# GrafikXxxxxxxYyyyyyyyyyy/StableDiffusion

Hardware: AMD Instinct MI355X
Metric: denoise-loop latents/s (512px, 50-step DDIM, batch 4) (higher is better)
Workload: dtype f16; 1 GPU; SD1.5 512x512, 50-step DDIM, batch 4/GPU, CFG on (UNet batch 8), UNet + VAE decode HIP kernels; global_batch=4, parallelism=dp1

## Files before the change

### stablediffusion_amd/build.py

```python
from __future__ import annotations

import os
import subprocess
import sys
from concurrent.futures import ThreadPoolExecutor

HERE = os.path.dirname(os.path.abspath(__file__))
CSRC = os.path.join(HERE, "csrc")
OUT = os.path.join(HERE, "libsd_engine.so")
SOURCES = ["igemm.hip", "igemm2.hip", "igemm3.hip", "wsgemm.hip", "pgemm.hip", "ffn.hip", "edge.hip", "norm.hip", "attention.hip", "ip_attention.hip", "controlnet.hip", "misc.hip", "probe.hip", "runtime.cpp", "unet.cpp", "controlnet.cpp", "vae.cpp", "clip.cpp", "capi.cpp"]
FLAGS = ["-O3", "--offload-arch=gfx950", "-fPIC", "-std=c++17", "-Wall", "-Wno-unused-function",
         "-ffp-contract=fast", "-mllvm", "-amdgpu-mfma-vgpr-form"]


def _stale(target, deps):
    if not os.path.exists(target):
        return True
    t = os.path.getmtime(target)
    return any(os.path.getmtime(d) > t for d in deps)


def build(force: bool = False, verbose: bool = False) -> str:
    hipcc = os.environ.get("HIPCC", "/opt/rocm/bin/hipcc")
    objdir = os.path.join(HERE, "build")
    os.makedirs(objdir, exist_ok=True)
    headers = [os.path.join(CSRC, f) for f in os.listdir(CSRC) if f.endswith((".h", ".inc"))]
    headers.append(os.path.join(os.path.dirname(HERE), "include", "sd_engine.h"))
    jobs = []
    objs = []
    for src in SOURCES:
        s = os.path.join(CSRC, src)
        o = os.path.join(objdir, src + ".o")
        objs.append(o)
        if force or _stale(o, [s] + headers):
            jobs.append([hipcc, *FLAGS, "-x", "hip", "-c", s, "-o", o])

    def run(cmd):
        if verbose:
            print(" ".join(cmd), flush=True)
        r = subprocess.run(cmd, capture_output=True, text=True)
        if r.returncode != 0:
            raise RuntimeError("build failed: %s\n%s\n%s" % (" ".join(cmd), r.stdout, r.stderr))
        if verbose and r.stderr.strip():
            print(r.stderr, file=sys.stderr)

    if jobs:
        with ThreadPoolExecutor(max_workers=min(8, len(jobs))) as ex:
            list(ex.map(run, jobs))
    if jobs or force or _stale(OUT, objs):
        run([hipcc, "--offload-arch=gfx950", "-shared", "-fPIC", "-o", OUT, *objs])
    return OUT


if __name__ == "__main__":
    print(build(force="--force" in sys.argv, verbose=True))
```

### stablediffusion_amd/csrc/attention.hip

```cpp
#include <cstdlib>

#include "kernels.h"

namespace sd {
namespace {

[[maybe_unused]] constexpr float kRescaleThreshold = 8.0f;

constexpr int odd32_bytes(int bytes) { return ((((bytes + 31) / 32) | 1)) * 32; }
constexpr int k_row_halves(int D) { return D == 40 ? 40 : odd32_bytes((D + 31) / 32 * 32 * 2) / 2; }

typedef __fp16 fp16x2 __attribute__((ext_vector_type(2)));

__device__ __forceinline__ unsigned pack_rtz(float a, float b) {
    return __builtin_bit_cast(unsigned, __builtin_amdgcn_cvt_pkrtz(a, b));
}

template <int D, int QT, int KT, bool PRESC, int NWV = 4>
__global__ __launch_bounds__(64 * NWV) void attn_kernel(const half_t* __restrict__ q,
                                                   const half_t* __restrict__ k,
                                                   const half_t* __restrict__ v,
                                                   half_t* __restrict__ out, int Tq, int Tk_all,
                                                   int heads, long ldq, long ldk, long ldv,
                                                   long ldo, float scale_log2e, int causal, int qblocks) {
    static_assert(KT == 64 || KT == 128, "keys per tile");
#if defined(__HIP_DEVICE_COMPILE__)
    constexpr int NSUB = KT / 16;
    constexpr int NKK = KT / 32;
    constexpr int DK = (D + 31) / 32 * 32;
    constexpr int KS = DK / 32;
    constexpr int DT = (D + 15) / 16 + ((D % 16 == 0 && D <= 64) ? 1 : 0);
    constexpr int KSTR = k_row_halves(D);
    constexpr int VSTR = odd32_bytes(DT * 16 * 2) / 2;
    constexpr int CH = D / 8;
    constexpr int NCH = KT * CH;
    constexpr bool ONES = DT * 16 > D;
    constexpr bool PREFETCH = D <= 160;
    constexpr int QB = 16 * QT * NWV;
    constexpr int NTH = 64 * NWV;

    constexpr int TILE_HALVES = KT * (KSTR + VSTR);
    extern __shared__ __attribute__((aligned(16))) char smem[];
    half_t* sK = reinterpret_cast<half_t*>(smem);
    half_t* sV = sK + KT * KSTR;

    const int tid = threadIdx.x, lane = tid & 63, wave = tid >> 6;
    const int fr = lane & 15, fq = lane >> 4;
    const int bid = xcd_remap(blockIdx.x, gridDim.x);
    const int bh = bid / qblocks, qblk = bid - bh * qblocks;
    const int b = bh / heads, h = bh - b * heads;
    const int q0 = qblk * QB + wave * (16 * QT);

    const half_t* qb = q + (long)b * Tq * ldq + h * D;
    int Tk = Tk_all;
    if (causal && qblk * QB + QB < Tk) Tk = qblk * QB + QB;
    const half_t* kb = k + (long)b * Tk_all * ldk + h * D;
    const half_t* vb = v + (long)b * Tk_all * ldv + h * D;

    constexpr int KPAD = KSTR - D, VPAD = VSTR - D;
#pragma unroll
    for (int bufi = 0; bufi < (PREFETCH ? 2 : 1); ++bufi) {
        if constexpr (KPAD > 0) {
            for (int idx = tid; idx < KT * KPAD; idx += NTH) {
                const int r = idx / KPAD, c = D + idx - r * KPAD;
                sK[bufi * TILE_HALVES + r * KSTR + c] = (half_t)0.f;
            }
        }
        if constexpr (VPAD > 0) {
            for (int idx = tid; idx < KT * VPAD; idx += NTH) {
                const int r = idx / VPAD, c = D + idx - r * VPAD;
                sV[bufi * TILE_HALVES + r * VSTR + c] = (ONES && c == D) ? (half_t)1.f : (half_t)0.f;
            }
        }
    }

    h8 qf[QT][KS];
#pragma unroll
    for (int t = 0; t < QT; ++t) {
        const int qi = q0 + t * 16 + fr;
#pragma unroll
        for (int ks = 0; ks < KS; ++ks) {
            const int c = ks * 32 + fq * 8;
            h8 val = {0, 0, 0, 0, 0, 0, 0, 0};
            if (qi < Tq && c < D) val = *reinterpret_cast<const h8*>(qb + (long)qi * ldq + c);
            qf[t][ks] = val;
        }
    }

    f4 o[DT][QT];
#pragma unroll
    for (int i = 0; i < DT; ++i)
#pragma unroll
        for (int t = 0; t < QT; ++t) o[i][t] = f4{0.f, 0.f, 0.f, 0.f};
    float mrun[QT], lrun[QT];
#pragma unroll
    for (int t = 0; t < QT; ++t) { mrun[t] = PRESC ? 0.f : -INFINITY; lrun[t] = 0.f; }
    f4 negm[QT];
#pragma unroll
    for (int t = 0; t < QT; ++t) negm[t] = f4{0.f, 0.f, 0.f, 0.f};

    constexpr unsigned kOOB = 0x80000000u;
    constexpr int SPRK = KSTR / 8, SPRV = VSTR / 8;
    constexpr int NP = SPRK + SPRV, NPW = (NP + NWV - 1) / NWV;
    const int wavu = __builtin_amdgcn_readfirstlane(wave);
    __amdgpu_buffer_rsrc_t rk = __builtin_amdgcn_make_buffer_rsrc(const_cast<half_t*>(kb), 0, 0x7fffffff, 0x00020000);
    __amdgpu_buffer_rsrc_t rv = __builtin_amdgcn_make_buffer_rsrc(const_cast<half_t*>(vb), 0, 0x7fffffff, 0x00020000);
    int p_row[NPW], p_off[NPW];
#pragma unroll
    for (int j = 0; j < NPW; ++j) {
        const int q = wavu + NWV * j;
        const bool isk = q < SPRK;
        const int spr = isk ? SPRK : SPRV;
        const int p = (isk ? q : q - SPRK) * 64 + lane;
        const int r = p / spr, c = p - r * spr;
        p_row[j] = r;
        p_off[j] = c < CH ? (int)((r * (isk ? ldk : ldv) + c * 8) * 2) : -1;
    }
    auto issue_tile = [&](int bufi, int kt0) {
        half_t* dK = sK + bufi * TILE_HALVES;
        half_t* dV = sV + bufi * TILE_HALVES;
        const unsigned kbase = (unsigned)((long)kt0 * ldk * 2), vbase = (unsigned)((long)kt0 * ldv * 2);
        const int lim = Tk - kt0;
#pragma unroll
        for (int j = 0; j < NPW; ++j) {
            const int q = wavu + NWV * j;
            if (q < NP && p_off[j] >= 0) {
                const bool isk = q < SPRK;
                const unsigned voff = p_row[j] < lim ? (isk ? kbase : vbase) + (unsigned)p_off[j] : kOOB;
                half_t* dst = isk ? dK + q * 512 : dV + (q - SPRK) * 512;
                if (isk)
                    __builtin_amdgcn_raw_ptr_buffer_load_lds(rk, (__attribute__((address_space(3))) void*)dst, 16, voff, 0, 0, 0);
                else
                    __builtin_amdgcn_raw_ptr_buffer_load_lds(rv, (__attribute__((address_space(3))) void*)dst, 16, voff, 0, 0, 0);
            }
        }
    };
    if (PREFETCH) {
        __syncthreads();
        issue_tile(0, 0);
        asm volatile("s_waitcnt vmcnt(0)" ::: "memory");
        __syncthreads();
    }

    int cur = 0;
    for (int kt0 = 0; kt0 < Tk; kt0 += KT) {
        if (PREFETCH) {
            if (kt0 + KT < Tk) issue_tile(cur ^ 1, kt0 + KT);
        } else {
            __syncthreads();
            for (int idx = tid; idx < NCH; idx += NTH) {
                const int r = idx / CH, c = (idx - r * CH) * 8;
                h8 kv = {0, 0, 0, 0, 0, 0, 0, 0}, vv = {0, 0, 0, 0, 0, 0, 0, 0};
                if (kt0 + r < Tk) {
                    kv = *reinterpret_cast<const h8*>(kb + (long)(kt0 + r) * ldk + c);
                    vv = *reinterpret_cast<const h8*>(vb + (long)(kt0 + r) * ldv + c);
                }
                *reinterpret_cast<h8*>(sK + r * KSTR + c) = kv;
                *reinterpret_cast<h8*>(sV + r * VSTR + c) = vv;
            }
            __syncthreads();
        }
        const half_t* cK = sK + cur * TILE_HALVES;
        const half_t* cV = sV + cur * TILE_HALVES;

        f4 s[NSUB][QT];
#pragma unroll
        for (int ksub = 0; ksub < NSUB; ++ksub)
#pragma unroll
            for (int t = 0; t < QT; ++t) s[ksub][t] = PRESC ? negm[t] : f4{0.f, 0.f, 0.f, 0.f};
#pragma unroll
        for (int ks = 0; ks < KS; ++ks) {
#pragma unroll
            for (int ksub = 0; ksub < NSUB; ++ksub) {
                const h8 kf = *reinterpret_cast<const h8*>(cK + (ksub * 16 + fr) * KSTR + ks * 32 + fq * 8);
#pragma unroll
                for (int t = 0; t < QT; ++t)
                    s[ksub][t] = __builtin_amdgcn_mfma_f32_16x16x32_f16(kf, qf[t][ks], s[ksub][t], 0, 0, 0);
            }
        }
        if (kt0 + KT > Tk) {
#pragma unroll
            for (int ksub = 0; ksub < NSUB; ++ksub)
#pragma unroll
                for (int j = 0; j < 4; ++j)
                    if (kt0 + ksub * 16 + fq * 4 + j >= Tk) {
#pragma unroll
                        for (int t = 0; t < QT; ++t) s[ksub][t][j] = -INFINITY;
                    }
        }

        if (causal && kt0 + KT - 1 > q0) {
#pragma unroll
            for (int t = 0; t < QT; ++t) {
                const int qi = q0 + t * 16 + fr;
#pragma unroll
                for (int ksub = 0; ksub < NSUB; ++ksub)
#pragma unroll
                    for (int j = 0; j < 4; ++j)
                        if (kt0 + ksub * 16 + fq * 4 + j > qi) s[ksub][t][j] = -INFINITY;
            }
        }

        unsigned pf[QT][NKK][4];
        if constexpr (PRESC) {
            float mx[QT];
            bool grow = kt0 == 0;
#pragma unroll
            for (int t = 0; t < QT; ++t) {
                float m = -INFINITY;
#pragma unroll
                for (int ksub = 0; ksub < NSUB; ++ksub)
#pragma unroll
                    for (int j = 0; j < 4; ++j) m = fmaxf(m, s[ksub][t][j]);
                mx[t] = m;
                grow |= m > kRescaleThreshold;
            }
            if (__any(grow)) {
#pragma unroll
                for (int t = 0; t < QT; ++t) {
                    mx[t] = fmaxf(mx[t], __shfl_xor(mx[t], 16));
                    mx[t] = fmaxf(mx[t], __shfl_xor(mx[t], 32));
                    const float delta = kt0 == 0 ? mx[t] : fmaxf(mx[t], 0.f);
                    const float alpha = kt0 == 0 ? 1.f : __builtin_amdgcn_exp2f(-delta);
                    mrun[t] += delta;
                    negm[t] = f4{-mrun[t], -mrun[t], -mrun[t], -mrun[t]};
#pragma unroll
                    for (int i = 0; i < DT; ++i) o[i][t] *= alpha;
                    lrun[t] *= alpha;
#pragma unroll
                    for (int ksub = 0; ksub < NSUB; ++ksub) s[ksub][t] -= delta;
                }
            }
#pragma unroll
            for (int t = 0; t < QT; ++t) {
                float psum = 0.f;
#pragma unroll
                for (int ksub = 0; ksub < NSUB; ++ksub) {
                    float p[4];
#pragma unroll
                    for (int j = 0; j < 4; ++j) {
                        p[j] = __builtin_amdgcn_exp2f(s[ksub][t][j]);
                        if (!ONES) psum += p[j];
                    }
                    pf[t][ksub >> 1][(ksub & 1) * 2] = pack_rtz(p[0], p[1]);
                    pf[t][ksub >> 1][(ksub & 1) * 2 + 1] = pack_rtz(p[2], p[3]);
                }
                if (!ONES) lrun[t] += psum;
            }
        } else {
            bool grow = false;
            float mx[QT];
    #pragma unroll
            for (int t = 0; t < QT; ++t) {
                float m = -INFINITY;
    #pragma unroll
                for (int ksub = 0; ksub < NSUB; ++ksub)
    #pragma unroll
                    for (int j = 0; j < 4; ++j) m = fmaxf(m, s[ksub][t][j]);
                m = fmaxf(m, __shfl_xor(m, 16));
                m = fmaxf(m, __shfl_xor(m, 32));
                mx[t] = m * scale_log2e;
                grow |= mx[t] > mrun[t] + kRescaleThreshold;
            }
            if (__any(grow)) {
    #pragma unroll
                for (int t = 0; t < QT; ++t) {
                    const float mnew = fmaxf(mrun[t], mx[t]);
                    const float alpha = __builtin_amdgcn_exp2f(mrun[t] - mnew);
                    mrun[t] = mnew;
                    lrun[t] *= alpha;
    #pragma unroll
                    for (int i = 0; i < DT; ++i) o[i][t] *= alpha;
                }
            }
    #pragma unroll
            for (int t = 0; t < QT; ++t) {
                const float nm = -mrun[t];
                float psum = 0.f;
    #pragma unroll
                for (int ksub = 0; ksub < NSUB; ++ksub) {
                    float p[4];
    #pragma unroll
                    for (int j = 0; j < 4; ++j) {
                        p[j] = __builtin_amdgcn_exp2f(__builtin_fmaf(s[ksub][t][j], scale_log2e, nm));
                        if (!ONES) psum += p[j];
                    }
                    pf[t][ksub >> 1][(ksub & 1) * 2] = pack_rtz(p[0], p[1]);
                    pf[t][ksub >> 1][(ksub & 1) * 2 + 1] = pack_rtz(p[2], p[3]);
                }
                if (!ONES) lrun[t] += psum;
            }
        }

#pragma unroll
        for (int i = 0; i < DT; ++i) {
#pragma unroll
            for (int kk = 0; kk < NKK; ++kk) {
                const half_t* a0 = cV + (kk * 32 + fq * 4 + (fr >> 2)) * VSTR + i * 16 + (fr & 3) * 4;
                const s4v lo = __builtin_amdgcn_ds_read_tr16_b64_v4i16(
                    (__attribute__((address_space(3))) s4v*)(a0));
                const s4v hi = __builtin_amdgcn_ds_read_tr16_b64_v4i16(
                    (__attribute__((address_space(3))) s4v*)(a0 + 16 * VSTR));
                union { struct { s4v a, b; } p; h8 v; } u;
                u.p.a = lo; u.p.b = hi;
#pragma unroll
                for (int t = 0; t < QT; ++t) {
                    union { unsigned w[4]; h8 v; } pb;
#pragma unroll
                    for (int e = 0; e < 4; ++e) pb.w[e] = pf[t][kk][e];
                    o[i][t] = __builtin_amdgcn_mfma_f32_16x16x32_f16(u.v, pb.v, o[i][t], 0, 0, 0);
                }
            }
        }
        if (PREFETCH) {
            asm volatile("s_waitcnt vmcnt(0)" ::: "memory");
            __syncthreads();
            cur ^= 1;
        }
    }

    half_t* ob = out + (long)b * Tq * ldo + h * D;
#pragma unroll
    for (int t = 0; t < QT; ++t) {
        float l;
        if (ONES) {
            constexpr int LT = D / 16, LQ = (D % 16) / 4, LJ = D % 4;
            l = __shfl(o[LT][t][LJ], LQ * 16 + fr);
        } else {
            l = lrun[t];
            l += __shfl_xor(l, 16);
            l += __shfl_xor(l, 32);
        }
        const float inv = 1.0f / l;
        const int qi = q0 + t * 16 + fr;
#pragma unroll
        for (int i = 0; i < DT; ++i) {
            const int dd = i * 16 + fq * 4;
            if (qi < Tq && dd < D) {
                const f4 val = o[i][t] * inv;
                h4 w = {(half_t)val[0], (half_t)val[1], (half_t)val[2], (half_t)val[3]};
                *reinterpret_cast<h4*>(ob + (long)qi * ldo + dd) = w;
            }
        }
    }
#endif
}

template <int D, int QT, int KT, bool PRESC, int NWV = 4>
int launch_attn(const half_t* q, const half_t* k, const half_t* v, half_t* out, int B, int Tq, int Tk,
                int heads, long ldq, long ldk, long ldv, long ldo, int causal, bool q_has_scale, hipStream_t s) {
    constexpr int DK = (D + 31) / 32 * 32;
    constexpr int DT = (D + 15) / 16 + ((D % 16 == 0 && D <= 64) ? 1 : 0);
    constexpr size_t lds = (size_t)KT * (k_row_halves(D) * 2 + odd32_bytes(DT * 16 * 2)) * (D <= 160 ? 2 : 1);
    static PerDeviceOnce attr_once;
    if (attr_once.first()) {
        SD_HIP_CHECK(hipFuncSetAttribute(reinterpret_cast<const void*>(&attn_kernel<D, QT, KT, PRESC, NWV>),
                                         hipFuncAttributeMaxDynamicSharedMemorySize, (int)lds));
    }
    const float scale_log2e = q_has_scale ? 1.0f : 1.4426950408889634f / sqrtf((float)D);
    const int qblocks = cdiv(Tq, 16 * QT * NWV);
    hipLaunchKernelGGL((attn_kernel<D, QT, KT, PRESC, NWV>), dim3(qblocks * B * heads), dim3(64 * NWV), lds, s, q, k, v,
                       out, Tq, Tk, heads, ldq, ldk, ldv, ldo, scale_log2e, causal, qblocks);
    SD_HIP_CHECK(hipGetLastError());
    return 0;
}

}

bool attention_supported(int d) {
    return d == 32 || d == 40 || d == 64 || d == 80 || d == 128 || d == 160 || d == 512;
}

int launch_attention(const half_t* q, const half_t* k, const half_t* v, half_t* out, int B, int Tq,
                     int Tk, int heads, int d, long ldq, long ldk, long ldv, long ldo, hipStream_t s, int causal,
                     int prescaled) {
    if ((ldq | ldk | ldv | ldo) % 8 != 0) { set_error("attention: row strides must be multiples of 8"); return 1; }
    if (Tk <= 0 || Tq <= 0) return 0;
#define SD_ATTN_CASE(DD, QQ, KK, FAST) \
    case DD: return (prescaled && FAST) \
        ? launch_attn<DD, QQ, KK, FAST>(q, k, v, out, B, Tq, Tk, heads, ldq, ldk, ldv, ldo, causal, true, s) \
        : launch_attn<DD, QQ, KK, false>(q, k, v, out, B, Tq, Tk, heads, ldq, ldk, ldv, ldo, causal, prescaled != 0, s)
    static const int nwv = getenv("SD_ATTN_NWV") ? atoi(getenv("SD_ATTN_NWV")) : 8;
    if (d == 40 && prescaled && !causal && nwv == 8 && (long)cdiv(Tq, 512) * B * heads >= 512)
        return launch_attn<40, 4, 64, true, 8>(q, k, v, out, B, Tq, Tk, heads, ldq, ldk, ldv, ldo, causal, true, s);
    static const int nwv80 = getenv("SD_ATTN_NWV80") ? atoi(getenv("SD_ATTN_NWV80")) : 8;
    if (nwv80 == 8 && !causal && d == 80 && (long)cdiv(Tq, 256) * B * heads >= 256)
        return launch_attn<80, 2, 64, false, 8>(q, k, v, out, B, Tq, Tk, heads, ldq, ldk, ldv, ldo, causal, prescaled != 0, s);
    if (d == 160 && (long)cdiv(Tq, 128) * B * heads < 256)
        return launch_attn<160, 1, 64, false>(q, k, v, out, B, Tq, Tk, heads, ldq, ldk, ldv, ldo, causal, prescaled != 0, s);
    switch (d) {
        SD_ATTN_CASE(32, 2, 64, true);
        SD_ATTN_CASE(40, 4, 64, true);
        SD_ATTN_CASE(64, 2, 64, false);
        SD_ATTN_CASE(80, 2, 64, false);
        SD_ATTN_CASE(128, 2, 64, false);
        SD_ATTN_CASE(160, 2, 64, false);
        SD_ATTN_CASE(512, 1, 64, false);
        default:
            set_error("attention: unsupported head dim " + std::to_string(d));
            return 4;
    }
#undef SD_ATTN_CASE
}

}
```

### stablediffusion_amd/csrc/kernels.h

```cpp
#pragma once
#include "common.h"

namespace sd {

struct IGemmParams {
    const half_t* x; long ldx;
    const half_t* w;
    const float* bias;
    const float* rowadd; int rowadd_ld;
    const half_t* res; long ldres;
    half_t* y; long ldy;
    int N, H, W, Cin;
    int OH, OW, Cout;
    int KS, stride, pad, up;
    int M, K;
    int geglu;
    int mfast = 0;
    int act = 0;
    float* rowstat_out = nullptr;
    int rowstat_parts = 0;
    const float* ln_stat = nullptr;
    int ln_parts = 0, ln_C = 0, ln_part_w = 0;
    float ln_eps = 0.f;
    const float* ln_wsum = nullptr;
    float* gnstat_out = nullptr;
    int gn_groups = 0;
    const float* gni_part = nullptr;
    int gni_S = 0;
    long gni_rows = 0;
    int gni_groups = 0;
    float gni_eps = 0.f;
    int gni_silu = 0;
    const float* gni_gb = nullptr;
    int dbg_unchecked = 0;
    float acc_scale = 1.f, bias_scale = 1.f;
};
bool igemm2_gn_fusable(const IGemmParams& p, int groups);
bool igemm2_scales_ok(const IGemmParams& p);
bool igemm2_emits_gnstats(const IGemmParams& p, int groups, int* rows);
bool igemm2_emits_rowstats(const IGemmParams& p, int* parts, int* part_w);
int launch_igemm(const IGemmParams& p, hipStream_t s);
const char* igemm_variant(const IGemmParams& p);
bool igemm2_supported(const IGemmParams& p);
void igemm2_pick(const IGemmParams& p, int* variant, int* splits);
const char* igemm2_name(int variant);
long igemm2_partial_floats(const IGemmParams& p);
int launch_igemm2(const IGemmParams& p, float* partial, hipStream_t s);
constexpr int kKindPgemmGeglu = 100;
int igemm2_launch_kind(const IGemmParams& p, bool have_partial);
void igemm2_force(int variant, int splits);
bool igemm3_supported(const IGemmParams& p);
int launch_igemm3(const IGemmParams& p, int mfast, hipStream_t s);
constexpr int kWeightRowPad = 256;
bool wsgemm_supported(const IGemmParams& p);
int wsgemm_rowstat_parts(const IGemmParams& p);
int launch_wsgemm(const IGemmParams& p, hipStream_t s);
bool pgemm_geglu_supported(const IGemmParams& p);
int launch_pgemm_geglu(const IGemmParams& p, hipStream_t s);

struct FfnParams {
    const half_t* x; long ldx;
    half_t* y; long ldy;
    const half_t* w1; const float* b1; const float* wsum1; int w1_rows;
    const half_t* w2; const float* b2; int w2_rows;
    const float* ln_stat; int ln_parts; float ln_eps;
    int M, C, hidden;
    int ln_part_w;
};
bool ffn_fused_supported(const FfnParams& p);
int launch_ffn_fused(const FfnParams& p, hipStream_t s);

long gn_scratch_floats(int N, long HW, int C, int G);
struct GnStats {
    const float* part = nullptr;
    int S = 0;
    long rows = 0;
};
bool gn_wants_stats(long HW, int C, int G);
int launch_groupnorm(const half_t* x, long ldx, const float* gamma, const float* beta,
                     half_t* y, long ldy, int N, long HW, int C, int G, float eps, int silu,
                     float* scratch, hipStream_t s, const GnStats* pre = nullptr);
int launch_gn_stats(const half_t* x, long ldx, int N, long HW, int C, int G, float* scratch, GnStats* st, hipStream_t s);
int launch_gn_finalize(GnStats* st, float* out, int N, long HW, int C, int G, hipStream_t s);
int gn_cat_unit(int Ca, int Cb, int G);
int launch_gn_cat_finalize(const GnStats& sa, int Ga, int Ca, const GnStats& sb, int Gb, int Cb, float* out, int N, long HW, int G,
                           hipStream_t s);
int launch_layernorm(const half_t* x, long ldx, const float* gamma, const float* beta,
                     half_t* y, long ldy, long rows, int C, float eps, hipStream_t s);
int launch_row_stats(const half_t* x, long ldx, float* stat, long rows, int C, hipStream_t s);
int launch_ln_fold(half_t* w, long K, int rows, const float* gamma, const float* beta, const float* bias_in,
                   float* bias, float* wsum, int rows_scaled, float row_scale, hipStream_t s);

int launch_attention(const half_t* q, const half_t* k, const half_t* v, half_t* out,
                     int B, int Tq, int Tk, int heads, int d,
                     long ldq, long ldk, long ldv, long ldo, hipStream_t s, int causal = 0, int prescaled = 0);
bool attention_supported(int d);
int launch_ip_attention(const half_t* q, const half_t* k, const half_t* v, const half_t* kip, const half_t* vip,
                        half_t* out, int B, int Tq, int L, int Tip, int heads, int d, long ldq, long ldk, long ldv,
                        long ldki, long ldvi, long ldo, float ip_scale, int prescaled, hipStream_t s);
bool ip_attention_supported(int d);
int launch_axpy_f16(half_t* y, long ldy, const half_t* x, long ldx, long rows, int cols, float a, hipStream_t s);

constexpr int kCnMaxProblems = 16;
struct CnResProblem {
    const half_t* x = nullptr; long ldx = 0;
    const half_t* w = nullptr;
    const float* bias = nullptr;
    half_t* y = nullptr; long ldy = 0;
    int M = 0, C = 0;
    int first = 0;
};
struct CnResParams {
    CnResProblem p[kCnMaxProblems];
    int count = 0, total = 0;
    float scale = 1.f;
};
int cn_residual_tiles(int M, int C);
bool cn_residual_supported(const CnResParams& p);
int launch_cn_residual(const CnResParams& p, hipStream_t s);
struct CnCondConvParams {
    const half_t* x = nullptr; int nchw = 0;
    const float* w = nullptr; const float* bias = nullptr;
    half_t* y = nullptr;
    int N = 0, IH = 0, IW = 0, Cin = 0, OH = 0, OW = 0, Cout = 0, stride = 1, silu = 1;
};
bool cn_cond_conv_supported(const CnCondConvParams& p);
int launch_cn_cond_conv(const CnCondConvParams& p, hipStream_t s);
int launch_cn_pack_cond(const half_t* w_oihw, float* out, int O, int I, hipStream_t s);

int launch_timestep_sinusoid(const float* t, int t_stride, float* out, int count, int dim, int flip, float shift,
                             long out_ld, hipStream_t s);
int launch_small_linear(const float* x, long ldx, const half_t* w, const float* bias, float* y,
                        long ldy, int B, int K, int Nout, int silu_in, int silu_out, hipStream_t s);
int launch_add_f32(float* y, const float* x, long n, int silu, hipStream_t s);
int launch_f16_to_f32(const half_t* x, float* y, long n, hipStream_t s);
int launch_f32_to_f16(const float* x, half_t* y, long n, hipStream_t s);
int launch_im2col_nchw3x3(const half_t* x, half_t* col, int N, int C, int H, int W, int Kpad,
                          hipStream_t s);
int launch_nhwc_to_nchw(const half_t* x, long ldx, half_t* y, int N, long HW, int C, hipStream_t s);
int launch_nchw_to_nhwc(const half_t* x, half_t* y, long ldy, int N, long HW, int C, hipStream_t s);
int launch_pointwise_nchw(const half_t* x, const half_t* w, const float* bias, half_t* y, int N,
                          int Cin, int Cout, long HW, hipStream_t s);
constexpr long kSmallCoutMinPixels = 131072;
int launch_conv3x3_small_cout(const half_t* x, long ldx, const half_t* w, long K, const float* bias, half_t* y_nchw,
                              int N, int H, int W, int Cin, int Cout, hipStream_t s);
struct HeadParams {
    const half_t* x_nchw = nullptr;
    const half_t* w = nullptr; long K = 0;
    const float* bias = nullptr;
    half_t* y = nullptr; long ldy = 0;
    float* gnstat_out = nullptr; int G = 0;
    int N = 0, Cin = 0, H = 0, W = 0, Cout = 0;
};
bool conv_head_supported(const HeadParams& p);
int launch_conv_head(const HeadParams& p, hipStream_t s);
struct TailParams {
    const half_t* x = nullptr; long ldx = 0;
    const float* gn_part = nullptr; int gn_S = 0; long gn_rows = 0;
    int G = 0; float eps = 0.f; const float* gamma = nullptr; const float* beta = nullptr; int silu = 0;
    const half_t* w = nullptr; long K = 0; const float* bias = nullptr;
    half_t* y = nullptr;
    int N = 0, H = 0, W = 0, C = 0, Cout = 0;
};
bool conv_tail_supported(const TailParams& p);
int launch_conv_tail(const TailParams& p, hipStream_t s);
int launch_pack_conv(const half_t* w_oihw, half_t* wp, int O, int I, int KH, int KW, long Kpad,
                     hipStream_t s);
int launch_cfg_duplicate(const half_t* lat, half_t* out, long n_total, float scale, hipStream_t s);
int launch_clip_embed(const int* ids, const half_t* tok, const half_t* pos, half_t* out, int B, int T, int H, int vocab,
                      hipStream_t s);
int launch_gather_rows(const half_t* x, long ldx, const int* idx, half_t* out16, float* out32, int B, int T, int H,
                       hipStream_t s);
int launch_inpaint_blend(half_t* lat, const half_t* img, const half_t* noise, const half_t* mask, float a, float b, int B,
                         int C, long HW, hipStream_t s);
int launch_scale_f16(half_t* x, long n, float scale, hipStream_t s);
int launch_image_to_uint8(const half_t* img, unsigned char* out, int B, int C, long HW, hipStream_t s);
int launch_cfg_linear(const half_t* eps2b, half_t* lat, float* hist, long n, float g, float cx, float ce, float ch,
                      float hx, float he, hipStream_t s);
int launch_cfg_ddim(const half_t* eps2b, half_t* lat, long n, float g, float cx, float ce,
                    hipStream_t s);

int probe_mfma(int iters, float* tflops, hipStream_t s);
int probe_copy(long bytes, int iters, float* gbs, hipStream_t s);
int probe_dma(long region_bytes, int passes, int depth, int shared, float* gbs, hipStream_t s);

}
```

Baseline: 7.860 latents/s.

## Add 32x32x16 MFMA flash-attention kernel for head dim 80 self-attention

After: 7.875 latents/s, median of 3. No clear change (+0.2%).

```diff
diff --git a/stablediffusion_amd/build.py b/stablediffusion_amd/build.py
--- a/stablediffusion_amd/build.py
+++ b/stablediffusion_amd/build.py
@@ -8,7 +8,7 @@
 HERE = os.path.dirname(os.path.abspath(__file__))
 CSRC = os.path.join(HERE, "csrc")
 OUT = os.path.join(HERE, "libsd_engine.so")
-SOURCES = ["igemm.hip", "igemm2.hip", "igemm3.hip", "wsgemm.hip", "pgemm.hip", "ffn.hip", "edge.hip", "norm.hip", "attention.hip", "ip_attention.hip", "controlnet.hip", "misc.hip", "probe.hip", "runtime.cpp", "unet.cpp", "controlnet.cpp", "vae.cpp", "clip.cpp", "capi.cpp"]
+SOURCES = ["igemm.hip", "igemm2.hip", "igemm3.hip", "wsgemm.hip", "pgemm.hip", "ffn.hip", "edge.hip", "norm.hip", "attention.hip", "attention32.hip", "ip_attention.hip", "controlnet.hip", "misc.hip", "probe.hip", "runtime.cpp", "unet.cpp", "controlnet.cpp", "vae.cpp", "clip.cpp", "capi.cpp"]
 FLAGS = ["-O3", "--offload-arch=gfx950", "-fPIC", "-std=c++17", "-Wall", "-Wno-unused-function",
          "-ffp-contract=fast", "-mllvm", "-amdgpu-mfma-vgpr-form"]
 
diff --git a/stablediffusion_amd/csrc/attention.hip b/stablediffusion_amd/csrc/attention.hip
--- a/stablediffusion_amd/csrc/attention.hip
+++ b/stablediffusion_amd/csrc/attention.hip
@@ -383,9 +383,10 @@
     static const int nwv = getenv("SD_ATTN_NWV") ? atoi(getenv("SD_ATTN_NWV")) : 8;
     if (d == 40 && prescaled && !causal && nwv == 8 && (long)cdiv(Tq, 512) * B * heads >= 512)
         return launch_attn<40, 4, 64, true, 8>(q, k, v, out, B, Tq, Tk, heads, ldq, ldk, ldv, ldo, causal, true, s);
-    static const int nwv80 = getenv("SD_ATTN_NWV80") ? atoi(getenv("SD_ATTN_NWV80")) : 8;
-    if (nwv80 == 8 && !causal && d == 80 && (long)cdiv(Tq, 256) * B * heads >= 256)
+    if (!causal && d == 80 && (long)cdiv(Tq, 256) * B * heads >= 256) {
+        if (Tk >= 256) return launch_attention32(q, k, v, out, B, Tq, Tk, heads, d, ldq, ldk, ldv, ldo, s, prescaled);
         return launch_attn<80, 2, 64, false, 8>(q, k, v, out, B, Tq, Tk, heads, ldq, ldk, ldv, ldo, causal, prescaled != 0, s);
+    }
     if (d == 160 && (long)cdiv(Tq, 128) * B * heads < 256)
         return launch_attn<160, 1, 64, false>(q, k, v, out, B, Tq, Tk, heads, ldq, ldk, ldv, ldo, causal, prescaled != 0, s);
     switch (d) {
diff --git a/stablediffusion_amd/csrc/attention32.hip b/stablediffusion_amd/csrc/attention32.hip
--- /dev/null
+++ b/stablediffusion_amd/csrc/attention32.hip
@@ -0,0 +1,343 @@
+#include "kernels.h"
+
+namespace sd {
+namespace {
+
+[[maybe_unused]] constexpr float kRescaleThreshold32 = 8.0f;
+
+struct Attn32Layout { int d, kstr, vw[3]; };
+constexpr Attn32Layout kAttn32Layouts[] = {
+    {80, 88, {32, 32, 32}},
+};
+constexpr Attn32Layout attn32_layout(int D) {
+    for (const Attn32Layout& l : kAttn32Layouts)
+        if (l.d == D) return l;
+    return Attn32Layout{0, 0, {0, 0, 0}};
+}
+constexpr int attn32_tile_halves(int D) {
+    const Attn32Layout l = attn32_layout(D);
+    return 64 * (l.kstr + l.vw[0] + l.vw[1] + l.vw[2]);
+}
+
+typedef float f16v __attribute__((ext_vector_type(16)));
+
+__device__ __forceinline__ unsigned pack_rtz32(float a, float b) {
+    return __builtin_bit_cast(unsigned, __builtin_amdgcn_cvt_pkrtz(a, b));
+}
+
+template <int D, int QN, bool PRESC, int NWV>
+__global__ __launch_bounds__(64 * NWV) void attn_kernel32(const half_t* __restrict__ q, const half_t* __restrict__ k,
+                                                     const half_t* __restrict__ v, half_t* __restrict__ out,
+                                                     int Tq, int Tk, int heads, long ldq, long ldk, long ldv,
+                                                     long ldo, float scale_log2e, int qblocks) {
+#if defined(__HIP_DEVICE_COMPILE__)
+    constexpr Attn32Layout L = attn32_layout(D);
+    static_assert(L.d == D && D % 8 == 0 && D % 32 != 0, "head dim without a layout row / without a spare PV row");
+    constexpr int KT = 64;
+    constexpr int KS = (D + 15) / 16;
+    constexpr int NVI = D / 32 + 1;
+    constexpr int KSTR = L.kstr;
+    constexpr int CH = D / 8;
+    constexpr int QB = 32 * QN * NWV, NTH = 64 * NWV;
+    constexpr int TILE_HALVES = attn32_tile_halves(D);
+    constexpr int VOFF[3] = {KT * KSTR, KT * (KSTR + L.vw[0]), KT * (KSTR + L.vw[0] + L.vw[1])};
+    static_assert(KSTR % 16 == 8 && KSTR >= KS * 16 - 8, "K stride: an odd number of 16-byte slots");
+    static_assert(L.vw[NVI - 1] > D % 32 && (NVI == 3 || L.vw[2] == 0), "last V image holds the ones column");
+
+    extern __shared__ __attribute__((aligned(16))) char smem[];
+    half_t* sT = reinterpret_cast<half_t*>(smem);
+
+    const int tid = threadIdx.x, lane = tid & 63, wave = tid >> 6;
+    const int r32 = lane & 31, hh = lane >> 5;
+    const int bid = xcd_remap(blockIdx.x, gridDim.x);
+    const int bh = bid / qblocks, qblk = bid - bh * qblocks;
+    const int b = bh / heads, h = bh - b * heads;
+    const int q0 = qblk * QB + wave * (32 * QN);
+
+    const half_t* qb = q + (long)b * Tq * ldq + h * D;
+    const half_t* kb = k + (long)b * Tk * ldk + h * D;
+    const half_t* vb = v + (long)b * Tk * ldv + h * D;
+
+#pragma unroll
+    for (int bufi = 0; bufi < 2; ++bufi)
+#pragma unroll
+        for (int i = 0; i < NVI; ++i) {
+            const int vw = L.vw[i];
+            if (32 * i + vw > D)
+                for (int idx = tid; idx < KT * vw; idx += NTH) {
+                    const int c = 32 * i + idx % vw;
+                    if (c >= D) sT[bufi * TILE_HALVES + VOFF[i] + idx] = c == D ? (half_t)1.f : (half_t)0.f;
+                }
+        }
+
+    h8 qf[QN][KS];
+#pragma unroll
+    for (int t = 0; t < QN; ++t) {
+        const int qi = q0 + t * 32 + r32;
+#pragma unroll
+        for (int ks = 0; ks < KS; ++ks) {
+            const int c = ks * 16 + hh * 8;
+            h8 val = {0, 0, 0, 0, 0, 0, 0, 0};
+            if (qi < Tq && c < D) val = *reinterpret_cast<const h8*>(qb + (long)qi * ldq + c);
+            qf[t][ks] = val;
+        }
+    }
+
+    f16v o[NVI][QN];
+#pragma unroll
+    for (int i = 0; i < NVI; ++i)
+#pragma unroll
+        for (int t = 0; t < QN; ++t)
+#pragma unroll
+            for (int e = 0; e < 16; ++e) o[i][t][e] = 0.f;
+    float mrun[QN];
+    f16v negm[QN];
+#pragma unroll
+    for (int t = 0; t < QN; ++t) {
+        mrun[t] = PRESC ? 0.f : -INFINITY;
+#pragma unroll
+        for (int e = 0; e < 16; ++e) negm[t][e] = 0.f;
+    }
+
+    constexpr unsigned kOOB = 0x80000000u;
+    constexpr int SPRK = KSTR / 8;
+    constexpr int NP = SPRK + (L.vw[0] + L.vw[1] + L.vw[2]) / 8, NPW = (NP + NWV - 1) / NWV;
+    const int wavu = __builtin_amdgcn_readfirstlane(wave);
+    __amdgpu_buffer_rsrc_t rk = __builtin_amdgcn_make_buffer_rsrc(const_cast<half_t*>(kb), 0, 0x7fffffff, 0x00020000);
+    __amdgpu_buffer_rsrc_t rv = __builtin_amdgcn_make_buffer_rsrc(const_cast<half_t*>(vb), 0, 0x7fffffff, 0x00020000);
+    int p_row[NPW], p_off[NPW], p_dst[NPW];
+#pragma unroll
+    for (int j = 0; j < NPW; ++j) {
+        const int pq = wavu + NWV * j;
+        int spr = SPRK, c0 = 0, dst = pq * 512, pin = pq;
+        if (pq >= SPRK) {
+            pin = pq - SPRK;
+#pragma unroll
+            for (int i = 0; i < NVI; ++i) {
+                const int n = L.vw[i] / 8;
+                if (pin >= 0 && pin < n) { spr = n; c0 = 4 * i; dst = VOFF[i] + pin * 512; break; }
+                pin -= n;
+            }
+        }
+        const int p = pin * 64 + lane;
+        const int r = p / spr, c = c0 + p - r * spr;
+        p_row[j] = r;
+        p_dst[j] = dst;
+        p_off[j] = c < CH ? (int)((r * (pq < SPRK ? ldk : ldv) + c * 8) * 2) : -1;
+    }
+    auto issue_tile = [&](int bufi, int kt0) {
+        half_t* dT = sT + bufi * TILE_HALVES;
+        const unsigned kbase = (unsigned)((long)kt0 * ldk * 2), vbase = (unsigned)((long)kt0 * ldv * 2);
+        const int lim = Tk - kt0;
+#pragma unroll
+        for (int j = 0; j < NPW; ++j) {
+            const int pq = wavu + NWV * j;
+            if (pq < NP && p_off[j] >= 0) {
+                const bool isk = pq < SPRK;
+                const unsigned voff = p_row[j] < lim ? (isk ? kbase : vbase) + (unsigned)p_off[j] : kOOB;
+                half_t* dst = dT + p_dst[j];
+                if (isk)
+                    __builtin_amdgcn_raw_ptr_buffer_load_lds(rk, (__attribute__((address_space(3))) void*)dst, 16, voff, 0, 0, 0);
+                else
+                    __builtin_amdgcn_raw_ptr_buffer_load_lds(rv, (__attribute__((address_space(3))) void*)dst, 16, voff, 0, 0, 0);
+            }
+        }
+    };
+    __syncthreads();
+    issue_tile(0, 0);
+    asm volatile("s_waitcnt vmcnt(0)" ::: "memory");
+    __syncthreads();
+
+    const int koff = r32 * KSTR + hh * 8;
+    int voff[NVI];
+#pragma unroll
+    for (int i = 0; i < NVI; ++i)
+        voff[i] = VOFF[i] + (hh * 4 + ((lane & 15) >> 2)) * L.vw[i] + (L.vw[i] == 32 ? (lane & 16) : 0) + (lane & 3) * 4;
+
+    int cur = 0;
+    for (int kt0 = 0; kt0 < Tk; kt0 += KT) {
+        if (kt0 + KT < Tk) issue_tile(cur ^ 1, kt0 + KT);
+        const half_t* cT = sT + cur * TILE_HALVES;
+
+        f16v s[2][QN];
+#pragma unroll
+        for (int kt = 0; kt < 2; ++kt)
+#pragma unroll
+            for (int t = 0; t < QN; ++t) {
+                if constexpr (PRESC) s[kt][t] = negm[t];
+                else
+#pragma unroll
+                    for (int e = 0; e < 16; ++e) s[kt][t][e] = 0.f;
+            }
+#pragma unroll
+        for (int ks = 0; ks < KS; ++ks) {
+#pragma unroll
+            for (int kt = 0; kt < 2; ++kt) {
+                const h8 kf = *reinterpret_cast<const h8*>(cT + koff + kt * 32 * KSTR + ks * 16);
+#pragma unroll
+                for (int t = 0; t < QN; ++t)
+                    s[kt][t] = __builtin_amdgcn_mfma_f32_32x32x16_f16(kf, qf[t][ks], s[kt][t], 0, 0, 0);
+            }
+        }
+        if (kt0 + KT > Tk) {
+#pragma unroll
+            for (int kt = 0; kt < 2; ++kt)
+#pragma unroll
+                for (int e = 0; e < 16; ++e)
+                    if (kt0 + kt * 32 + (e & 3) + 8 * (e >> 2) + 4 * hh >= Tk) {
+#pragma unroll
+                        for (int t = 0; t < QN; ++t) s[kt][t][e] = -INFINITY;
+                    }
+        }
+
+        unsigned pf[QN][2][2][4];
+        if constexpr (PRESC) {
+            float mx[QN];
+            bool grow = kt0 == 0;
+#pragma unroll
+            for (int t = 0; t < QN; ++t) {
+                float m = -INFINITY;
+#pragma unroll
+                for (int kt = 0; kt < 2; ++kt)
+#pragma unroll
+                    for (int e = 0; e < 16; ++e) m = fmaxf(m, s[kt][t][e]);
+                mx[t] = m;
+                grow |= m > kRescaleThreshold32;
+            }
+            if (__any(grow)) {
+#pragma unroll
+                for (int t = 0; t < QN; ++t) {
+                    mx[t] = fmaxf(mx[t], __shfl_xor(mx[t], 32));
+                    const float delta = kt0 == 0 ? mx[t] : fmaxf(mx[t], 0.f);
+                    const float alpha = kt0 == 0 ? 1.f : __builtin_amdgcn_exp2f(-delta);
+                    mrun[t] += delta;
+#pragma unroll
+                    for (int e = 0; e < 16; ++e) negm[t][e] = -mrun[t];
+#pragma unroll
+                    for (int i = 0; i < NVI; ++i) o[i][t] *= alpha;
+#pragma unroll
+                    for (int kt = 0; kt < 2; ++kt) s[kt][t] -= delta;
+                }
+            }
+#pragma unroll
+            for (int t = 0; t < QN; ++t)
+#pragma unroll
+                for (int kt = 0; kt < 2; ++kt)
+#pragma unroll
+                    for (int e = 0; e < 8; ++e)
+                        pf[t][kt][e >> 2][e & 3] = pack_rtz32(__builtin_amdgcn_exp2f(s[kt][t][2 * e]),
+                                                              __builtin_amdgcn_exp2f(s[kt][t][2 * e + 1]));
+        } else {
+            bool grow = false;
+            float mx[QN];
+#pragma unroll
+            for (int t = 0; t < QN; ++t) {
+                float m = -INFINITY;
+#pragma unroll
+                for (int kt = 0; kt < 2; ++kt)
+#pragma unroll
+                    for (int e = 0; e < 16; ++e) m = fmaxf(m, s[kt][t][e]);
+                m = fmaxf(m, __shfl_xor(m, 32));
+                mx[t] = m * scale_log2e;
+                grow |= mx[t] > mrun[t] + kRescaleThreshold32;
+            }
+            if (__any(grow)) {
+#pragma unroll
+                for (int t = 0; t < QN; ++t) {
+                    const float mnew = fmaxf(mrun[t], mx[t]);
+                    const float alpha = __builtin_amdgcn_exp2f(mrun[t] - mnew);
+                    mrun[t] = mnew;
+#pragma unroll
+                    for (int i = 0; i < NVI; ++i) o[i][t] *= alpha;
+                }
+            }
+#pragma unroll
+            for (int t = 0; t < QN; ++t) {
+                const float nm = -mrun[t];
+#pragma unroll
+                for (int kt = 0; kt < 2; ++kt)
+#pragma unroll
+                    for (int e = 0; e < 8; ++e)
+                        pf[t][kt][e >> 2][e & 3] =
+                            pack_rtz32(__builtin_amdgcn_exp2f(__builtin_fmaf(s[kt][t][2 * e], scale_log2e, nm)),
+                                       __builtin_amdgcn_exp2f(__builtin_fmaf(s[kt][t][2 * e + 1], scale_log2e, nm)));
+            }
+        }
+
+#pragma unroll
+        for (int i = 0; i < NVI; ++i) {
+#pragma unroll
+            for (int kt = 0; kt < 2; ++kt)
+#pragma unroll
+                for (int s2 = 0; s2 < 2; ++s2) {
+                    const half_t* a0 = cT + voff[i] + (kt * 32 + s2 * 16) * L.vw[i];
+                    const s4v lo = __builtin_amdgcn_ds_read_tr16_b64_v4i16(
+                        (__attribute__((address_space(3))) s4v*)(a0));
+                    const s4v hi = __builtin_amdgcn_ds_read_tr16_b64_v4i16(
+                        (__attribute__((address_space(3))) s4v*)(a0 + 8 * L.vw[i]));
+                    union { struct { s4v a, b; } p; h8 v; } u;
+                    u.p.a = lo; u.p.b = hi;
+#pragma unroll
+                    for (int t = 0; t < QN; ++t) {
+                        union { unsigned w[4]; h8 v; } pb;
+#pragma unroll
+                        for (int e = 0; e < 4; ++e) pb.w[e] = pf[t][kt][s2][e];
+                        o[i][t] = __builtin_amdgcn_mfma_f32_32x32x16_f16(u.v, pb.v, o[i][t], 0, 0, 0);
+                    }
+                }
+        }
+        asm volatile("s_waitcnt vmcnt(0)" ::: "memory");
+        __syncthreads();
+        cur ^= 1;
+    }
+
+    half_t* ob = out + (long)b * Tq * ldo + h * D;
+    constexpr int R = D % 32, LI = D / 32, LH = (R >> 2) & 1, LE = (R & 3) + 4 * (R >> 3);
+#pragma unroll
+    for (int t = 0; t < QN; ++t) {
+        const float l = __shfl(o[LI][t][LE], LH * 32 + r32);
+        const float inv = 1.0f / l;
+        const int qi = q0 + t * 32 + r32;
+#pragma unroll
+        for (int i = 0; i < NVI; ++i)
+#pragma unroll
+            for (int g = 0; g < 4; ++g) {
+                const int dd = i * 32 + g * 8 + hh * 4;
+                if (qi < Tq && dd < D) {
+                    h4 w = {(half_t)(o[i][t][4 * g] * inv), (half_t)(o[i][t][4 * g + 1] * inv),
+                            (half_t)(o[i][t][4 * g + 2] * inv), (half_t)(o[i][t][4 * g + 3] * inv)};
+                    *reinterpret_cast<h4*>(ob + (long)qi * ldo + dd) = w;
+                }
+            }
+    }
+#endif
+}
+
+template <int D, int QN, bool PRESC, int NWV>
+int launch_attn32(const half_t* q, const half_t* k, const half_t* v, half_t* out, int B, int Tq, int Tk, int heads,
+                  long ldq, long ldk, long ldv, long ldo, bool q_has_scale, hipStream_t s) {
+    constexpr size_t lds = (size_t)attn32_tile_halves(D) * 2 * 2;
+    static PerDeviceOnce attr_once;
+    if (attr_once.first()) {
+        SD_HIP_CHECK(hipFuncSetAttribute(reinterpret_cast<const void*>(&attn_kernel32<D, QN, PRESC, NWV>),
+                                         hipFuncAttributeMaxDynamicSharedMemorySize, (int)lds));
+    }
+    const float scale_log2e = q_has_scale ? 1.0f : 1.4426950408889634f / sqrtf((float)D);
+    const int qblocks = cdiv(Tq, 32 * QN * NWV);
+    hipLaunchKernelGGL((attn_kernel32<D, QN, PRESC, NWV>), dim3(qblocks * B * heads), dim3(64 * NWV), lds, s, q, k, v,
+                       out, Tq, Tk, heads, ldq, ldk, ldv, ldo, scale_log2e, qblocks);
+    SD_HIP_CHECK(hipGetLastError());
+    return 0;
+}
+
+}
+
+int launch_attention32(const half_t* q, const half_t* k, const half_t* v, half_t* out, int B, int Tq, int Tk,
+                       int heads, int d, long ldq, long ldk, long ldv, long ldo, hipStream_t s, int prescaled) {
+    if (d == 80)
+        return launch_attn32<80, 1, false, 8>(q, k, v, out, B, Tq, Tk, heads, ldq, ldk, ldv, ldo, prescaled != 0, s);
+    set_error("attention32: no 32x32x16 form for head dim " + std::to_string(d));
+    return 4;
+}
+
+}
diff --git a/stablediffusion_amd/csrc/kernels.h b/stablediffusion_amd/csrc/kernels.h
--- a/stablediffusion_amd/csrc/kernels.h
+++ b/stablediffusion_amd/csrc/kernels.h
@@ -95,6 +95,8 @@
                      int B, int Tq, int Tk, int heads, int d,
                      long ldq, long ldk, long ldv, long ldo, hipStream_t s, int causal = 0, int prescaled = 0);
 bool attention_supported(int d);
+int launch_attention32(const half_t* q, const half_t* k, const half_t* v, half_t* out, int B, int Tq, int Tk,
+                       int heads, int d, long ldq, long ldk, long ldv, long ldo, hipStream_t s, int prescaled);
 int launch_ip_attention(const half_t* q, const half_t* k, const half_t* v, const half_t* kip, const half_t* vip,
                         half_t* out, int B, int Tq, int L, int Tip, int heads, int d, long ldq, long ldk, long ldv,
                         long ldki, long ldvi, long ldo, float ip_scale, int prescaled, hipStream_t s);
```
